# pagmerek/frave

Measured on AMD Instinct MI355X. Metric: Mpixels/s encode (transform+quant) at 4096x4096, higher is better.
Workload: dtype u8->i32

## Files before the change

### frave_amd/csrc/k4_fit.hip

```cpp
#include "gather_common.hpp"
#include "solve6.hpp"

namespace fri {
namespace {

__device__ __forceinline__ uint32_t f32_to_u32_sat(float x) {
    uint32_t r;
    asm("v_cvt_u32_f32 %0, %1" : "=v"(r) : "v"(x));
    return r;
}

struct FitArgs {
    const int32_t *coefs;
    const int32_t *pred_slots;
    const uint16_t *nbr_table;
    const uint8_t *interior;
    const uint32_t *valid_mask;
    uint32_t n_tiles;
    PredictParams pp;
    const uint32_t *pred_off;
    const uint16_t *pair_pos;
    const uint32_t *halo_list;
    unsigned long long *gram;
    unsigned long long *wtw;
    double *wtr;
    unsigned long long *out_range;
    unsigned long long *acc;
    size_t coef_stride;
    const PredictParams *params;
    PredictParams pp3[3];
    int32_t ablate;
    unsigned long long *trace;
    int32_t older_eighths;
    float *solve_params;
    float *host_params;
    unsigned long long *host_range;
    unsigned long long rows[3];
};
constexpr int kFitAccInt = 3 * 28, kFitAccDbl = kFitAccInt, kFitAccTicket = kFitAccInt + 18, kFitAccRange = kFitAccTicket + 1;
static_assert(kFitAccRange + 1 == (int)kFitAccWords, "fit accumulator layout");

template <int OFFSET>
__device__ __forceinline__ void fit2_gather(uint32_t (&g)[6], const uint32_t (&a)[6], const uint32_t (&b)[6]) {
    uint32_t lo[6], hi[6];
    asm volatile("ds_read_u16 %0, %12 offset:%24\n\t"
                 "ds_read_u16 %1, %13 offset:%24\n\t"
                 "ds_read_u16 %2, %14 offset:%24\n\t"
                 "ds_read_u16 %3, %15 offset:%24\n\t"
                 "ds_read_u16 %4, %16 offset:%24\n\t"
                 "ds_read_u16 %5, %17 offset:%24\n\t"
                 "ds_read_u16_d16_hi %6, %18 offset:%24\n\t"
                 "ds_read_u16_d16_hi %7, %19 offset:%24\n\t"
                 "ds_read_u16_d16_hi %8, %20 offset:%24\n\t"
                 "ds_read_u16_d16_hi %9, %21 offset:%24\n\t"
                 "ds_read_u16_d16_hi %10, %22 offset:%24\n\t"
                 "ds_read_u16_d16_hi %11, %23 offset:%24\n\t"
                 "s_waitcnt lgkmcnt(0)"
                 : "=&v"(lo[0]), "=&v"(lo[1]), "=&v"(lo[2]), "=&v"(lo[3]), "=&v"(lo[4]), "=&v"(lo[5]), "=&v"(hi[0]), "=&v"(hi[1]), "=&v"(hi[2]), "=&v"(hi[3]), "=&v"(hi[4]),
                   "=&v"(hi[5])
                 : "v"(a[0]), "v"(a[1]), "v"(a[2]), "v"(a[3]), "v"(a[4]), "v"(a[5]), "v"(b[0]), "v"(b[1]), "v"(b[2]), "v"(b[3]), "v"(b[4]), "v"(b[5]), "n"(OFFSET)
                 : "memory");
#pragma unroll
    for (int k = 0; k < 6; k++) g[k] = lo[k] | hi[k];
}

template <int OFFSET>
__device__ __forceinline__ void fit2_gather_floats(uint32_t (&lo)[6], uint32_t (&hi)[6], const uint32_t (&a)[6], const uint32_t (&b)[6]) {
    asm volatile("ds_read_u16_d16_hi %0, %12 offset:%24\n\t"
                 "ds_read_u16_d16_hi %1, %13 offset:%24\n\t"
                 "ds_read_u16_d16_hi %2, %14 offset:%24\n\t"
                 "ds_read_u16_d16_hi %3, %15 offset:%24\n\t"
                 "ds_read_u16_d16_hi %4, %16 offset:%24\n\t"
                 "ds_read_u16_d16_hi %5, %17 offset:%24\n\t"
                 "ds_read_u16_d16_hi %6, %18 offset:%24\n\t"
                 "ds_read_u16_d16_hi %7, %19 offset:%24\n\t"
                 "ds_read_u16_d16_hi %8, %20 offset:%24\n\t"
                 "ds_read_u16_d16_hi %9, %21 offset:%24\n\t"
                 "ds_read_u16_d16_hi %10, %22 offset:%24\n\t"
                 "ds_read_u16_d16_hi %11, %23 offset:%24\n\t"
                 "s_waitcnt lgkmcnt(0)"
                 : "=&v"(lo[0]), "=&v"(lo[1]), "=&v"(lo[2]), "=&v"(lo[3]), "=&v"(lo[4]), "=&v"(lo[5]), "=&v"(hi[0]), "=&v"(hi[1]), "=&v"(hi[2]), "=&v"(hi[3]), "=&v"(hi[4]),
                   "=&v"(hi[5])
                 : "v"(a[0]), "v"(a[1]), "v"(a[2]), "v"(a[3]), "v"(a[4]), "v"(a[5]), "v"(b[0]), "v"(b[1]), "v"(b[2]), "v"(b[3]), "v"(b[4]), "v"(b[5]), "n"(OFFSET)
                 : "memory");
}

__device__ __forceinline__ void fit2_pair_value(const uint32_t (&g)[6], uint32_t own, int (&acc)[28]) {
    s16x2 u[7];
#pragma unroll
    for (int k = 0; k < 6; k++) u[k] = __builtin_bit_cast(s16x2, g[k]);
    u[6] = __builtin_bit_cast(s16x2, own);
    int n = 0;
#pragma unroll
    for (int r0 = 0; r0 < 7; r0++)
#pragma unroll
        for (int c0 = r0; c0 < 7; c0++, n++) acc[n] = __builtin_amdgcn_sdot2(u[r0], u[c0], acc[n], false);
}

__device__ __forceinline__ void fit2_pair_width(const uint32_t (&lo)[6], const uint32_t (&hi)[6], uint32_t own, uint32_t one_bits, const float (&vp)[6], int (&acc)[28],
                                                float (&facc)[6]) {
    float fa[7], fb[7];
#pragma unroll
    for (int k = 0; k < 6; k++) fa[k] = __builtin_bit_cast(float, lo[k]), fb[k] = __builtin_bit_cast(float, hi[k]);
    fa[6] = __builtin_bit_cast(float, own << 16), fb[6] = __builtin_bit_cast(float, own & 0xFFFF0000u);
    float pa = __fmul_rn(fa[0], vp[0]), pb = __fmul_rn(fb[0], vp[0]);
#pragma unroll
    for (int k = 1; k < 6; k++) pa = __fadd_rn(pa, __fmul_rn(fa[k], vp[k])), pb = __fadd_rn(pb, __fmul_rn(fb[k], vp[k]));
    const float ra = fabsf(__fsub_rn(fa[6], pa)), rb = fabsf(__fsub_rn(fb[6], pb));
    constexpr int kD0[5] = {0, 1, 4, 1, 2}, kD1[5] = {3, 2, 5, 5, 4};
    float da[5], db[5];
#pragma unroll
    for (int j = 0; j < 5; j++) da[j] = fabsf(__fsub_rn(fa[kD0[j]], fa[kD1[j]])), db[j] = fabsf(__fsub_rn(fb[kD0[j]], fb[kD1[j]]));
    s16x2 w[6];
    w[0] = __builtin_bit_cast(s16x2, one_bits);
#pragma unroll
    for (int j = 0; j < 5; j++) {
        const uint32_t ia = __builtin_bit_cast(uint32_t, __fadd_rn(da[j], 8388608.0f)), ib = __builtin_bit_cast(uint32_t, __fadd_rn(db[j], 8388608.0f));
        w[1 + j] = __builtin_bit_cast(s16x2, __builtin_amdgcn_perm(ib, ia, 0x05040100u));
    }
    int n = 0;
#pragma unroll
    for (int r0 = 0; r0 < 6; r0++)
#pragma unroll
        for (int c0 = r0; c0 < 6; c0++, n++) acc[n] = __builtin_amdgcn_sdot2(w[r0], w[c0], acc[n], false);
    facc[0] = __fadd_rn(__fadd_rn(facc[0], ra), rb);
#pragma unroll
    for (int j = 0; j < 5; j++) {
        facc[1 + j] = __builtin_fmaf(da[j], ra, facc[1 + j]);
        facc[1 + j] = __builtin_fmaf(db[j], rb, facc[1 + j]);
    }
}

constexpr int kFit2Slot = 1024;
constexpr int kFit2Image = kPredSlots * kFit2Slot;
static_assert(kFit2Image + (kPredSide + kPredBlock) * kFit2Slot < 65536, "image + cell offset must fit a DS instruction's offset field");
struct Fit2Block {
    int4 lo, hi;
};
__device__ __forceinline__ int fit2_block_slot(int wave, int i) {
    const int c = 2 * wave + i;
    return (1 + c / kPredBlock) * kPredSide + 1 + (c % kPredBlock);
}
template <bool C16 = false>
__device__ __forceinline__ void fit2_block_load(Fit2Block &r, const int32_t *__restrict__ coefs, const int32_t *s_slot_cell, int slot, int lane, bool skip) {
    r.lo = make_int4(0, 0, 0, 0), r.hi = r.lo;
    const int cell = skip ? -1 : s_slot_cell[slot];
    if (cell >= 0) {
        if (C16) {
            r.lo = *reinterpret_cast<const int4 *>(reinterpret_cast<const int16_t *>(coefs) + (size_t)cell * kCell + 8 * lane);
        } else {
            const int4 *src = reinterpret_cast<const int4 *>(coefs + (size_t)cell * kCell + 8 * lane);
            r.lo = src[0];
            r.hi = src[1];
        }
    }
}
template <bool FLOATS>
__device__ __forceinline__ uint32_t fit2_pack(int first, int second) {
    if (!FLOATS) return __builtin_amdgcn_perm((uint32_t)second, (uint32_t)first, 0x05040100u);
    return __builtin_amdgcn_perm(__builtin_bit_cast(uint32_t, (float)(short)second), __builtin_bit_cast(uint32_t, (float)(short)first), 0x07060302u);
}
template <bool CHECK, bool FLOATS, bool C16 = false>
__device__ __forceinline__ void fit2_block_commit(const Fit2Block &r, const int32_t *s_slot_cell, uint8_t *image, int slot, int lane, uint32_t stage_pos, uint32_t *range_counter) {
    auto pk = [](int lo16, int hi16) -> uint32_t { return fit2_pack<FLOATS>(lo16, hi16); };
    if (C16) {
        static_assert(!(C16 && CHECK), "compact planes come from this library's forward kernel: nothing to check");
        auto pair = [&](int d) -> uint32_t { return FLOATS ? fit2_pack<true>(d, d >> 16) : (uint32_t)d; };
        uint8_t *dst = image + slot * kFit2Slot;
        *reinterpret_cast<uint32_t *>(dst + 4u * (stage_pos & 255u)) = pair(r.lo.x) & (lane == 0 ? 0xFFFF0000u : 0xFFFFFFFFu);
        *reinterpret_cast<uint32_t *>(dst + 4u * ((stage_pos >> 8) & 255u)) = pair(r.lo.y);
        *reinterpret_cast<uint32_t *>(dst + 4u * ((stage_pos >> 16) & 255u)) = pair(r.lo.z);
        *reinterpret_cast<uint32_t *>(dst + 4u * (stage_pos >> 24)) = pair(r.lo.w);
        return;
    }
    const int4 lo = r.lo, hi = r.hi;
    if (CHECK && s_slot_cell[slot] >= 0) {
        const int v[8] = {lo.x, lo.y, lo.z, lo.w, hi.x, hi.y, hi.z, hi.w};
        uint32_t m = 0;
#pragma unroll
        for (int j = 0; j < 8; j++) m |= v[j] == kNone ? 0u : ((uint32_t)v[j] + 256u) & 0xFFFFFE00u;
        if (__any(m != 0) && lane == 0) atomicAdd(range_counter, 1u);
    }
    uint8_t *dst = image + slot * kFit2Slot;
    *reinterpret_cast<uint32_t *>(dst + 4u * (stage_pos & 255u)) = pk(lo.x, lo.y) & (lane == 0 ? 0xFFFF0000u : 0xFFFFFFFFu);
    *reinterpret_cast<uint32_t *>(dst + 4u * ((stage_pos >> 8) & 255u)) = pk(lo.z, lo.w);
    *reinterpret_cast<uint32_t *>(dst + 4u * ((stage_pos >> 16) & 255u)) = pk(hi.x, hi.y);
    *reinterpret_cast<uint32_t *>(dst + 4u * (stage_pos >> 24)) = pk(hi.z, hi.w);
}
template <bool C16 = false>
__device__ __forceinline__ int fit2_halo_load(const int32_t *__restrict__ coefs, const int32_t *s_slot_cell, uint32_t entry, bool skip) {
    const int cell = skip ? -1 : s_slot_cell[entry & 63u];
    if (C16) return cell >= 0 ? (int)reinterpret_cast<const int16_t *>(coefs)[(size_t)cell * kCell + ((entry >> 8) & 511u)] : 0;
    return cell >= 0 ? coefs[(size_t)cell * kCell + ((entry >> 8) & 511u)] : 0;
}
template <bool FLOATS>
__device__ __forceinline__ void fit2_halo_commit(int v, uint8_t *image, uint32_t entry) {
    const uint16_t h = FLOATS ? (uint16_t)(__builtin_bit_cast(uint32_t, (float)(short)v) >> 16) : (uint16_t)v;
    *reinterpret_cast<uint16_t *>(image + (entry & 63u) * kFit2Slot + (entry >> 20)) = h;
}

template <int MODE, int IMG, int C>
__device__ __forceinline__ void fit2_cell(const int32_t *s_slot_cell, uint32_t has_bits, uint32_t interior_bits, const uint32_t *mask_word, uint32_t mask_shift, uint32_t keep, int slot0,
                                          const uint32_t (&addr)[2][6], uint32_t own_addr, const float (&vp)[6], int (&acc)[28], float (&facc)[6]) {
    constexpr int kBit = (C >> 2) * kPredSide + (C & 3);
    constexpr int kOff = IMG * kFit2Image + kBit * kFit2Slot;
    if (!((has_bits >> kBit) & 1u)) return;
    uint32_t own = *(__attribute__((address_space(3))) const uint32_t *)(uintptr_t)(own_addr + kOff) & keep;
    uint32_t one = keep & 0x00010001u;
    const bool boundary = !((interior_bits >> kBit) & 1u);
    if (MODE == 0) {
        uint32_t g[6];
        fit2_gather<kOff>(g, addr[0], addr[1]);
        if (boundary) {
            const int cell = __builtin_amdgcn_readfirstlane(s_slot_cell[slot0 + kBit]);
            const uint32_t bits = mask_word[(size_t)cell * 16] >> mask_shift;
            const uint32_t mask = ((bits & 1u) ? 0x0000FFFFu : 0u) | ((bits & 2u) ? 0xFFFF0000u : 0u);
#pragma unroll
            for (int k = 0; k < 6; k++) g[k] &= mask;
            own &= mask;
        }
        fit2_pair_value(g, own, acc);
    } else {
        uint32_t lo[6], hi[6];
        fit2_gather_floats<kOff>(lo, hi, addr[0], addr[1]);
        if (boundary) {
            const int cell = __builtin_amdgcn_readfirstlane(s_slot_cell[slot0 + kBit]);
            const uint32_t bits = mask_word[(size_t)cell * 16] >> mask_shift;
            const uint32_t first = (bits & 1u) ? 0xFFFFFFFFu : 0u, second = (bits & 2u) ? 0xFFFFFFFFu : 0u;
#pragma unroll
            for (int k = 0; k < 6; k++) lo[k] &= first, hi[k] &= second;
            own &= (first & 0xFFFFu) | (second << 16), one &= (first & 0xFFFFu) | (second << 16);
        }
        fit2_pair_width(lo, hi, own, one, vp, acc, facc);
    }
    asm volatile("" ::: "memory");
}
template <int MODE, int IMG, int C0>
__device__ __forceinline__ void fit2_cells(const int32_t *s_slot_cell, uint32_t has_bits, uint32_t interior_bits, const uint32_t *mask_word, uint32_t mask_shift, uint32_t keep, int slot0,
                                           const uint32_t (&addr)[2][6], uint32_t own_addr, const float (&vp)[6], int (&acc)[28], float (&facc)[6]) {
    fit2_cell<MODE, IMG, C0 + 0>(s_slot_cell, has_bits, interior_bits, mask_word, mask_shift, keep, slot0, addr, own_addr, vp, acc, facc);
    fit2_cell<MODE, IMG, C0 + 1>(s_slot_cell, has_bits, interior_bits, mask_word, mask_shift, keep, slot0, addr, own_addr, vp, acc, facc);
    fit2_cell<MODE, IMG, C0 + 2>(s_slot_cell, has_bits, interior_bits, mask_word, mask_shift, keep, slot0, addr, own_addr, vp, acc, facc);
    fit2_cell<MODE, IMG, C0 + 3>(s_slot_cell, has_bits, interior_bits, mask_word, mask_shift, keep, slot0, addr, own_addr, vp, acc, facc);
}

template <int NI>
__device__ __forceinline__ void fit2_wave_sums(int (&acc)[28], int group, int lane, unsigned long long (*s_int)[28]) {
    int r[NI];
#pragma unroll
    for (int k = 0; k < NI; k++) r[k] = acc[k], acc[k] = 0;
#pragma unroll
    for (int k = 0; k < NI; k++) r[k] += __builtin_amdgcn_update_dpp(0, r[k], 0xB1, 0xF, 0xF, true);
#pragma unroll
    for (int k = 0; k < NI; k++) r[k] += __builtin_amdgcn_update_dpp(0, r[k], 0x4E, 0xF, 0xF, true);
#pragma unroll
    for (int k = 0; k < NI; k++) r[k] += __builtin_amdgcn_update_dpp(0, r[k], 0x141, 0xF, 0xF, true);
#pragma unroll
    for (int k = 0; k < NI; k++) r[k] += __builtin_amdgcn_update_dpp(0, r[k], 0x140, 0xF, 0xF, true);
    if ((lane & 15) == 0) {
        unsigned long long *const mine = &s_int[(lane >> 4) * 3 + group][0];
#pragma unroll
        for (int k = 0; k < NI; k++) atomicAdd(mine + k, (unsigned long long)(long long)r[k]);
    }
}

constexpr int kFitFixBits = 20;
__device__ __forceinline__ unsigned long long fit_f32_to_fixed(float v0, bool &saturated) {
    saturated = saturated || !(v0 < 16777216.0f);
    const float v = fminf(v0, 16777216.0f);
    const float t = __builtin_truncf(v);
    const uint32_t hi = f32_to_u32_sat(t);
    const uint32_t lo = f32_to_u32_sat((v - t) * (float)(1u << kFitFixBits));
    return ((unsigned long long)hi << kFitFixBits) + lo;
}

template <int MODE>
__device__ __attribute__((noinline)) void fit2_tail_solve(const long long *sums_int, const double *sums_dbl, unsigned long long rows, Solve6Work *w, float *params,
                                                          float *host_params) {
    float out[6];
    if (MODE == 0)
        fit_value_group(sums_int, out, *w);
    else
        fit_width_group(sums_int, sums_dbl, rows, out, *w);
#pragma unroll
    for (int k = 0; k < 6; k++) params[k] = out[k];
    if (host_params) {
#pragma unroll
        for (int k = 0; k < 6; k++) host_params[k] = out[k];
    }
}

template <int MODE, bool CHECK, bool C16 = false>
__global__ void __launch_bounds__(kPredThreads, 4) fit_accumulate_kernel2(const FitArgs a0) {
    constexpr int NI = MODE == 0 ? 28 : 21;
    const uint32_t plane = blockIdx.y;
    const int32_t *const coefs = C16 ? reinterpret_cast<const int32_t *>(reinterpret_cast<const int16_t *>(a0.coefs) + plane * a0.coef_stride) : a0.coefs + plane * a0.coef_stride;
    unsigned long long *const accp = a0.acc + (size_t)plane * kFitShards * kFitAccWords;
    unsigned long long *const accs = accp + (size_t)(blockIdx.x % kFitShards) * kFitAccWords;
    PredictParams pp;
    if (a0.params)
        pp = a0.params[plane];
    else if (plane == 0)
        pp = a0.pp3[0];
    else if (plane == 1)
        pp = a0.pp3[1];
    else
        pp = a0.pp3[2];
    __shared__ __attribute__((aligned(16))) uint8_t s_cells[2 * kFit2Image];
    __shared__ int32_t s_slot_cell[2][kPredSlots];
    __shared__ uint32_t s_slot_bits[2][2];
    __shared__ uint32_t s_flag, s_range;
    __shared__ unsigned long long s_int[4 * 3][28];
    __shared__ unsigned long long s_fix[16 * 3][6];
    __shared__ double s_dbl[3][6];
    const int tid = threadIdx.x, lane = tid & 63;
    const int wave = __builtin_amdgcn_readfirstlane(tid >> 6);
    const int pg = wave & 3, half = wave >> 2;
    const int n0 = pg == 0 ? 128 + 2 * lane : pg == 1 ? 2 * lane : 256 + 4 * lane + 2 * (pg & 1);
    const int ablate = ablate_flags(a0.ablate);
    PredTileWalk walk(a0.n_tiles);
    if (a0.older_eighths > 0 && gridDim.x >= 16u && gridDim.x % 16u == 0u) {
        const uint32_t per_xcd = gridDim.x / 8u, pairs = per_xcd / 2u;
        const uint32_t xcd = blockIdx.x % 8u, in_xcd = blockIdx.x / 8u, pair = in_xcd % pairs, younger = in_xcd / pairs;
        const uint32_t lo = (uint32_t)((uint64_t)a0.n_tiles * xcd / 8u), hi = (uint32_t)((uint64_t)a0.n_tiles * (xcd + 1u) / 8u);
        const uint32_t n_pair = lo + pair < hi ? (hi - lo - pair + pairs - 1u) / pairs : 0u;
        const uint32_t n_older = min(n_pair, (n_pair * (uint32_t)a0.older_eighths + 3u) / 8u);
        walk.step = pairs;
        walk.first = lo + pair + (younger ? n_older * pairs : 0u);
        walk.end = younger ? hi : min(hi, lo + pair + n_older * pairs);
        if (walk.first > walk.end) walk.first = walk.end;
    }
    auto slot_entry = [&](uint32_t t) {
        uint32_t off = (uint32_t)tid * 4u;
        asm volatile("" : "+v"(off));
        return *reinterpret_cast<const int32_t *>(reinterpret_cast<const uint8_t *>(a0.pred_slots + (size_t)t * kPredSlots) + off);
    };
    const u32x4 off_a = reinterpret_cast<const u32x4 *>(a0.pred_off)[n0], off_b = reinterpret_cast<const u32x4 *>(a0.pred_off)[n0 + 1];
    const uint32_t own_pos = a0.pair_pos[n0 >> 1];
    const uint32_t halo_e0 = a0.halo_list[tid], halo_e1 = a0.halo_list[tid + kPredThreads];
    const uint32_t stage_pos = (uint32_t)a0.pair_pos[4 * lane] | (uint32_t)a0.pair_pos[4 * lane + 1] << 8 | (uint32_t)a0.pair_pos[4 * lane + 2] << 16 | (uint32_t)a0.pair_pos[4 * lane + 3] << 24;
    int first_raw = -1, next_raw = -1;
    if (tid < kPredSlots && walk.first < walk.end) first_raw = slot_entry(walk.first);
    if (tid < kPredSlots && walk.first + walk.step < walk.end) next_raw = slot_entry(walk.first + walk.step);
    __builtin_amdgcn_sched_barrier(0);
    if (tid < 4 * 3 * 28) (&s_int[0][0])[tid] = 0;
    if (tid < 16 * 18) (&s_fix[0][0])[tid] = 0ull;
    if (tid == 0) s_range = 0;
    trace_stamp(a0.trace, blockIdx.x, 0, tid);

    const int group = pg == 0 ? 1 : pg == 1 ? 2 : 0;
    const int slot0 = (1 + 2 * half) * kPredSide + 1;
    const uint32_t cells_lds = (uint32_t)(uintptr_t)(__attribute__((address_space(3))) uint8_t *)s_cells;
    uint32_t addr[2][6];
#pragma unroll
    for (int j = 0; j < 2; j++) {
        const u32x4 o = j == 0 ? off_a : off_b;
        const uint32_t rel[3] = {o.x, o.y, o.z};
#pragma unroll
        for (int k = 0; k < 6; k++) {
            const int r = (int)(short)((rel[k >> 1] >> (16 * (k & 1))) & 0xFFFFu);
            addr[j][k] = cells_lds + (uint32_t)(slot0 * kFit2Slot + (r == 0x7FFF ? 0 : r));
        }
    }
    uint32_t own_addr = cells_lds + (uint32_t)(slot0 * kFit2Slot) + 4u * own_pos;
    if (n0 == 0) {
#pragma unroll
        for (int j = 0; j < 2; j++)
#pragma unroll
            for (int k = 0; k < 6; k++) addr[j][k] = cells_lds + (uint32_t)(slot0 * kFit2Slot);
    }
    const uint32_t *const mask_word = a0.valid_mask + (n0 >> 5);
    const uint32_t mask_shift = n0 & 31;
    const uint32_t keep = n0 == 0 ? 0u : 0xFFFFFFFFu;
    float vp[6];
#pragma unroll
    for (int k = 0; k < 6; k++) vp[k] = group == 0 ? pp.value[0][k] : group == 1 ? pp.value[1][k] : pp.value[2][k];
    int acc[28];
    unsigned long long fx[6];
#pragma unroll
    for (int k = 0; k < 28; k++) acc[k] = 0;
#pragma unroll
    for (int k = 0; k < 6; k++) fx[k] = 0ull;
    bool fx_saturated = false;
    int tiles_since_flush = 0, trace_it = 0;
    const int block_a = fit2_block_slot(wave, 0), block_b = fit2_block_slot(wave, 1);

    uint32_t tile = walk.first;
    static_assert((kPredBlock * kPredSide + kPredBlock) < 32 && kPredSlots <= 64, "the block slots' bits fit one word; the slot table is written by one wave");
    auto slot_table = [&](int img, int raw) {
        s_slot_cell[img][tid] = pred_slot_cell(raw);
        const unsigned long long has = __ballot(pred_slot_cell(raw) >= 0), interior = __ballot(pred_slot_interior(raw));
        if (tid == 0) s_slot_bits[img][0] = (uint32_t)has, s_slot_bits[img][1] = (uint32_t)interior;
    };
#define FRI_FIT2_PHASE(IMG)                                                                                                                       \
    {                                                                                                                                            \
               \
                                                          \
        if (tid < kPredSlots) slot_table(IMG ^ 1, tile + walk.step < walk.end ? next_raw : -1);                                                  \
        __syncthreads();                                                                                                                         \
        float facc[6] = {0.f, 0.f, 0.f, 0.f, 0.f, 0.f};                                                                                          \
        const uint32_t has_bits = (uint32_t)__builtin_amdgcn_readfirstlane((int)s_slot_bits[IMG][0]) >> slot0;                                   \
        const uint32_t interior_bits = (uint32_t)__builtin_amdgcn_readfirstlane((int)s_slot_bits[IMG][1]) >> slot0;                              \
        {                                                                                                                                        \
            Fit2Block st;                                                                                                                        \
            fit2_block_load<C16>(st, coefs, s_slot_cell[IMG ^ 1], block_a, lane, ablate & 2);                                                         \
            const int hv = fit2_halo_load<C16>(coefs, s_slot_cell[IMG ^ 1], halo_e0, ablate & 2);                                                     \
            if (tid < kPredSlots && tile + 2 * walk.step < walk.end) next_raw = slot_entry(tile + 2 * walk.step);                                 \
            if (!(ablate & 1)) fit2_cells<MODE, IMG, 0>(s_slot_cell[IMG], has_bits, interior_bits, mask_word, mask_shift, keep, slot0, addr, own_addr, vp, acc, facc); \
            fit2_block_commit<CHECK, MODE == 1, C16>(st, s_slot_cell[IMG ^ 1], s_cells + (IMG ^ 1) * kFit2Image, block_a, lane, stage_pos, &s_range);                              \
            fit2_halo_commit<MODE == 1>(hv, s_cells + (IMG ^ 1) * kFit2Image, halo_e0);                                                                     \
        }                                                                                                                                        \
        {                                                                                                                                        \
            Fit2Block st;                                                                                                                        \
            fit2_block_load<C16>(st, coefs, s_slot_cell[IMG ^ 1], block_b, lane, ablate & 2);                                                         \
            const int hv = fit2_halo_load<C16>(coefs, s_slot_cell[IMG ^ 1], halo_e1, ablate & 2);                                                     \
            if (!(ablate & 1)) fit2_cells<MODE, IMG, 4>(s_slot_cell[IMG], has_bits, interior_bits, mask_word, mask_shift, keep, slot0, addr, own_addr, vp, acc, facc); \
            fit2_block_commit<CHECK, MODE == 1, C16>(st, s_slot_cell[IMG ^ 1], s_cells + (IMG ^ 1) * kFit2Image, block_b, lane, stage_pos, &s_range);                              \
            fit2_halo_commit<MODE == 1>(hv, s_cells + (IMG ^ 1) * kFit2Image, halo_e1);                                                                     \
        }                                                                                                                                        \
        if (MODE == 1) {                                                                                                                         \
            _Pragma("unroll") for (int k = 0; k < 6; k++) fx[k] += fit_f32_to_fixed(facc[k], fx_saturated);                                     \
        }                                                                                                                                        \
        if (++tiles_since_flush >= 16) {             \
            fit2_wave_sums<NI>(acc, group, lane, s_int);                                                                                         \
            tiles_since_flush = 0;                                                                                                               \
        }                                                                                                                                        \
        __syncthreads();                                                                                                                         \
        trace_stamp(a0.trace, blockIdx.x, 2 + trace_it++, tid);                                                                                  \
        tile += walk.step;                                                                                                                       \
    }
    if (tile < walk.end) {
        if (tid < kPredSlots) slot_table(0, first_raw);
        __syncthreads();
        {
            Fit2Block sa, sb;
            fit2_block_load<C16>(sa, coefs, s_slot_cell[0], block_a, lane, false);
            fit2_block_load<C16>(sb, coefs, s_slot_cell[0], block_b, lane, false);
            const int h0 = fit2_halo_load<C16>(coefs, s_slot_cell[0], halo_e0, false), h1 = fit2_halo_load<C16>(coefs, s_slot_cell[0], halo_e1, false);
            fit2_block_commit<CHECK, MODE == 1, C16>(sa, s_slot_cell[0], s_cells, block_a, lane, stage_pos, &s_range);
            fit2_block_commit<CHECK, MODE == 1, C16>(sb, s_slot_cell[0], s_cells, block_b, lane, stage_pos, &s_range);
            fit2_halo_commit<MODE == 1>(h0, s_cells, halo_e0);
            fit2_halo_commit<MODE == 1>(h1, s_cells, halo_e1);
        }
        __syncthreads();
        trace_stamp(a0.trace, blockIdx.x, 1, tid);
        while (true) {
            FRI_FIT2_PHASE(0)
            if (tile >= walk.end) break;
            FRI_FIT2_PHASE(1)
            if (tile >= walk.end) break;
        }
    }
#undef FRI_FIT2_PHASE
    trace_stamp(a0.trace, blockIdx.x, 13, tid);
    fit2_wave_sums<NI>(acc, group, lane, s_int);
    if (MODE == 1) {
        unsigned long long *const mine = &s_fix[(lane & 15) * 3 + group][0];
#pragma unroll
        for (int k = 0; k < 6; k++) atomicAdd(mine + k, fx[k]);
        if (__any(fx_saturated) && lane == 0) atomicAdd(&s_range, 1u);
    }
    __syncthreads();
    if (tid < 3 * NI) {
        const int gg = tid / NI, k = tid % NI;
        __hip_atomic_fetch_add(accs + tid, (s_int[gg][k] + s_int[3 + gg][k]) + (s_int[6 + gg][k] + s_int[9 + gg][k]), __ATOMIC_RELAXED, __HIP_MEMORY_SCOPE_AGENT);
    }
    if (MODE == 1 && tid < 18) {
        unsigned long long v = 0;
#pragma unroll
        for (int c = 0; c < 16; c++) v += (&s_fix[0][0])[c * 18 + tid];
        __hip_atomic_fetch_add(accs + kFitAccDbl + tid, v, __ATOMIC_RELAXED, __HIP_MEMORY_SCOPE_AGENT);
    }
    if (tid == 0 && s_range) __hip_atomic_fetch_add(accp + kFitAccRange, (unsigned long long)s_range, __ATOMIC_RELAXED, __HIP_MEMORY_SCOPE_AGENT);
    wait_for_own_memory_ops_then_barrier();
    if (tid == 0) s_flag = __hip_atomic_fetch_add(accp + kFitAccTicket, 1ull, __ATOMIC_RELAXED, __HIP_MEMORY_SCOPE_AGENT) == gridDim.x - 1 ? 1u : 0u;
    __syncthreads();
    trace_exit(a0.trace, blockIdx.x, tid);
    if (s_flag == 0) return;
    if (tid >= 64) return;
    unsigned long long *const out_int = (MODE == 0 ? a0.gram : a0.wtw) + (size_t)plane * 3 * NI;
    for (int i = tid; i < 3 * NI; i += 64) {
        unsigned long long part[kFitShards], sum = 0;
#pragma unroll
        for (uint32_t sh = 0; sh < kFitShards; sh++) part[sh] = __hip_atomic_load(accp + sh * kFitAccWords + i, __ATOMIC_RELAXED, __HIP_MEMORY_SCOPE_AGENT);
#pragma unroll
        for (uint32_t sh = 0; sh < kFitShards; sh++) {
            sum += part[sh];
            __hip_atomic_store(accp + sh * kFitAccWords + i, 0ull, __ATOMIC_RELAXED, __HIP_MEMORY_SCOPE_AGENT);
        }
        out_int[i] = sum;
        s_int[i / NI][i % NI] = sum;
    }
    if (MODE == 1 && tid < 18) {
        unsigned long long part[kFitShards], total = 0;
#pragma unroll
        for (uint32_t sh = 0; sh < kFitShards; sh++) part[sh] = __hip_atomic_load(accp + sh * kFitAccWords + kFitAccDbl + tid, __ATOMIC_RELAXED, __HIP_MEMORY_SCOPE_AGENT);
#pragma unroll
        for (uint32_t sh = 0; sh < kFitShards; sh++) {
            total += part[sh];
            __hip_atomic_store(accp + sh * kFitAccWords + kFitAccDbl + tid, 0ull, __ATOMIC_RELAXED, __HIP_MEMORY_SCOPE_AGENT);
        }
        const double sum = (double)total * (1.0 / (double)(1ull << kFitFixBits));
        a0.wtr[(size_t)plane * 18 + tid] = sum;
        (&s_dbl[0][0])[tid] = sum;
    }
    if (tid == 0) {
        const unsigned long long r = __hip_atomic_exchange(accp + kFitAccRange, 0ull, __ATOMIC_RELAXED, __HIP_MEMORY_SCOPE_AGENT);
        if (a0.out_range) a0.out_range[plane] = r;
        if (a0.host_range) a0.host_range[plane] = r;
        __hip_atomic_store(accp + kFitAccTicket, 0ull, __ATOMIC_RELAXED, __HIP_MEMORY_SCOPE_AGENT);
    }
    if (!a0.solve_params) return;
    __builtin_amdgcn_fence(__ATOMIC_RELEASE, "wavefront");
    __builtin_amdgcn_wave_barrier();
    __builtin_amdgcn_fence(__ATOMIC_ACQUIRE, "wavefront");
    if (tid < 3) {
        static_assert(3 * sizeof(Solve6Work) <= 2 * kFit2Image, "the solve's workspace lives in the cell images");
        const unsigned long long rows = tid == 0 ? a0.rows[0] : tid == 1 ? a0.rows[1] : a0.rows[2];
        const size_t at = (size_t)plane * (sizeof(PredictParams) / sizeof(float)) + (MODE ? 18 : 0) + tid * 6;
        fit2_tail_solve<MODE>(reinterpret_cast<const long long *>(s_int[tid]), s_dbl[tid], rows, reinterpret_cast<Solve6Work *>(s_cells) + tid, a0.solve_params + at,
                              a0.host_params ? a0.host_params + at : nullptr);
    }
}

struct SolveArgs {
    const unsigned long long *sums_int;
    const double *sums_dbl;
    float *params;
    uint32_t n_planes;
    unsigned long long rows[3];
    float *host_params;
    const unsigned long long *range;
    unsigned long long *host_range;
};
constexpr uint32_t kSolveThreads = 32;
template <int MODE>
__global__ void __launch_bounds__(kSolveThreads) fit_solve_kernel(const SolveArgs a) {
    __shared__ Solve6Work s_work[kSolveThreads];
    Solve6Work &w = s_work[threadIdx.x];
    const uint32_t t = blockIdx.x * kSolveThreads + threadIdx.x;
    if (t >= a.n_planes * 3u) return;
    const uint32_t plane = t / 3u, g = t % 3u;
    float *out = a.params + (size_t)plane * (sizeof(PredictParams) / sizeof(float)) + (MODE ? 18 : 0) + g * 6;
    if (MODE == 0) {
        fit_value_group(reinterpret_cast<const long long *>(a.sums_int) + ((size_t)plane * 3 + g) * 28, out, w);
    } else {
        const unsigned long long rows = g == 0 ? a.rows[0] : g == 1 ? a.rows[1] : a.rows[2];
        fit_width_group(reinterpret_cast<const long long *>(a.sums_int) + ((size_t)plane * 3 + g) * 21, a.sums_dbl + ((size_t)plane * 3 + g) * 6, rows, out, w);
    }
    if (a.host_params) {
        float *h = a.host_params + (out - a.params);
#pragma unroll
        for (int k = 0; k < 6; k++) h[k] = out[k];
        if (g == 0 && a.range && a.host_range) a.host_range[plane] = a.range[plane];
    }
}

}

hipError_t launch_fit_solve(int mode, uint32_t n_planes, const unsigned long long *sums_int, const double *sums_dbl, const unsigned long long rows[3], float *params,
                            hipStream_t stream, float *host_params, const unsigned long long *range, unsigned long long *host_range) {
    if (!n_planes || !sums_int || !params || (mode == 1 && !sums_dbl)) return hipErrorInvalidValue;
    SolveArgs a{};
    a.sums_int = sums_int;
    a.sums_dbl = sums_dbl;
    a.params = params;
    a.n_planes = n_planes;
    a.host_params = host_params, a.range = range, a.host_range = host_range;
    for (int g = 0; g < 3; g++) a.rows[g] = rows ? rows[g] : 0;
    const uint32_t blocks = (n_planes * 3u + kSolveThreads - 1u) / kSolveThreads;
    (void)hipGetLastError();
    if (mode == 0)
        hipLaunchKernelGGL(fit_solve_kernel<0>, dim3(blocks), dim3(kSolveThreads), 0, stream, a);
    else
        hipLaunchKernelGGL(fit_solve_kernel<1>, dim3(blocks), dim3(kSolveThreads), 0, stream, a);
    return hipGetLastError();
}

hipError_t launch_fit_accumulate(const DevicePlan &p, unsigned long long *acc, int mode, const PredBatch &b, unsigned long long *sums_int, double *sums_dbl,
                                 unsigned long long *out_of_range, hipStream_t stream, const FitSolve *solve, int trust) {
    if (!acc || !b.n_planes || b.n_planes > 65535u) return hipErrorInvalidValue;
    FitArgs a{};
    if (b.coefs16 && trust != kPredForwardOutput) return hipErrorInvalidValue;
    a.coefs = b.coefs16 ? reinterpret_cast<const int32_t *>(b.coefs16) : b.coefs;
    a.coef_stride = b.coef_stride;
    a.params = b.params;
    for (int k = 0; k < 3; k++) a.pp3[k] = b.pp[k];
    a.pred_slots = p.pred_slots;
    a.nbr_table = p.nbr_table;
    a.pred_off = p.gather_off;
    a.pair_pos = p.pair_pos;
    a.halo_list = p.halo_list;
    a.interior = p.interior;
    a.valid_mask = p.valid_mask;
    a.n_tiles = p.n_pred_tiles;
    a.acc = acc;
    a.gram = sums_int;
    a.wtw = sums_int;
    a.wtr = sums_dbl;
    a.out_range = out_of_range;
    if (solve) {
        if (!solve->params) return hipErrorInvalidValue;
        a.solve_params = solve->params, a.host_params = solve->host_params, a.host_range = solve->host_range;
        for (int g = 0; g < 3; g++) a.rows[g] = solve->rows[g];
    }
    a.ablate = p.k4_ablate;
    a.trace = p.trace;
    a.older_eighths = b.n_planes == 1 && p.hist_blocks <= p.n_pred_tiles ? p.k4_older_eighths : 0;
    uint32_t blocks = p.n_pred_tiles < p.hist_blocks ? p.n_pred_tiles : p.hist_blocks;
    if (b.n_planes > 1) {
        const uint32_t share = (p.n_pred_tiles + 7) / 8, eighth = p.hist_blocks / 8 ? p.hist_blocks / 8 : 1;
        blocks = share < eighth ? eighth : share;
        if (blocks > p.hist_blocks) blocks = p.hist_blocks;
        if (blocks > p.n_pred_tiles) blocks = p.n_pred_tiles;
    }
    if (!blocks) blocks = 1;
    (void)hipGetLastError();
    const bool check = trust != kPredForwardOutput;
    void (*kern)(const FitArgs) = mode == 0 ? (check ? fit_accumulate_kernel2<0, true> : fit_accumulate_kernel2<0, false>) : (check ? fit_accumulate_kernel2<1, true> : fit_accumulate_kernel2<1, false>);
    if (b.coefs16) kern = mode == 0 ? fit_accumulate_kernel2<0, false, true> : fit_accumulate_kernel2<1, false, true>;
    hipLaunchKernelGGL(kern, dim3(blocks, b.n_planes), dim3(kPredThreads), 0, stream, a);
    return hipGetLastError();
}

}
```

### frave_amd/csrc/solve6.hpp

```cpp
#pragma once
#include <cmath>

#if defined(__HIPCC__)
#define FRI_HD __host__ __device__
#else
#define FRI_HD
#endif

namespace fri {

struct Solve6Work {
    double m[6][6], y[6], x[6];
    double l[6][6], d[6], inv[6], z[6];
    double a[6][6], v[6][6];
};

#if defined(__HIP_DEVICE_COMPILE__)
#define FRI_SOLVE_STAGE() asm volatile("" ::: "memory")
#else
#define FRI_SOLVE_STAGE() ((void)0)
#endif

FRI_HD inline void solve6(Solve6Work &w) {
    {
        double dmax = 0.0;
#pragma unroll
        for (int i = 0; i < 6; i++) dmax = w.m[i][i] > dmax ? w.m[i][i] : dmax;
        bool ok = dmax > 0.0 && dmax < 1.0e300;
        FRI_SOLVE_STAGE();
#pragma unroll
        for (int j = 0; j < 6; j++) {
            double dj = w.m[j][j];
#pragma unroll
            for (int k = 0; k < j; k++) dj -= w.l[j][k] * w.l[j][k] * w.d[k];
            ok = ok && dj > 1e-8 * dmax;
            w.d[j] = dj;
            w.inv[j] = 1.0 / dj;
#pragma unroll
            for (int i = j + 1; i < 6; i++) {
                double t = w.m[i][j];
#pragma unroll
                for (int k = 0; k < j; k++) t -= w.l[i][k] * w.l[j][k] * w.d[k];
                w.l[i][j] = t * w.inv[j];
            }
            FRI_SOLVE_STAGE();
        }
        if (ok) {
#pragma unroll
            for (int i = 0; i < 6; i++) {
                double t = w.y[i];
#pragma unroll
                for (int k = 0; k < i; k++) t -= w.l[i][k] * w.z[k];
                w.z[i] = t;
            }
            FRI_SOLVE_STAGE();
#pragma unroll
            for (int i = 5; i >= 0; i--) {
                double t = w.z[i] * w.inv[i];
#pragma unroll
                for (int k = i + 1; k < 6; k++) t -= w.l[k][i] * w.x[k];
                w.x[i] = t;
            }
            return;
        }
    }
#pragma unroll 1
    for (int i = 0; i < 6; i++)
#pragma unroll 1
        for (int j = 0; j < 6; j++) {
            w.a[i][j] = w.m[i][j];
            w.v[i][j] = i == j ? 1.0 : 0.0;
        }
#pragma unroll 1
    for (int sweep = 0; sweep < 60; sweep++) {
        double off = 0.0;
#pragma unroll 1
        for (int i = 0; i < 6; i++)
#pragma unroll 1
            for (int j = i + 1; j < 6; j++) off += w.a[i][j] * w.a[i][j];
        if (!(off >= 1e-300)) break;
#pragma unroll 1
        for (int pp = 0; pp < 6; pp++)
#pragma unroll 1
            for (int q = pp + 1; q < 6; q++) {
                const double apq = w.a[pp][q];
                if ((apq < 0 ? -apq : apq) < 1e-300) continue;
                const double theta = (w.a[q][q] - w.a[pp][pp]) / (2.0 * apq);
                const double t = (theta >= 0 ? 1.0 : -1.0) / ((theta < 0 ? -theta : theta) + sqrt(theta * theta + 1.0));
                const double c = 1.0 / sqrt(t * t + 1.0), sn = t * c;
#pragma unroll 1
                for (int k = 0; k < 6; k++) {
                    const double akp = w.a[k][pp], akq = w.a[k][q];
                    w.a[k][pp] = c * akp - sn * akq;
                    w.a[k][q] = sn * akp + c * akq;
                }
#pragma unroll 1
                for (int k = 0; k < 6; k++) {
                    const double apk = w.a[pp][k], aqk = w.a[q][k];
                    w.a[pp][k] = c * apk - sn * aqk;
                    w.a[q][k] = sn * apk + c * aqk;
                }
#pragma unroll 1
                for (int k = 0; k < 6; k++) {
                    const double vkp = w.v[k][pp], vkq = w.v[k][q];
                    w.v[k][pp] = c * vkp - sn * vkq;
                    w.v[k][q] = sn * vkp + c * vkq;
                }
            }
    }
    double lmax = 0.0;
#pragma unroll 1
    for (int i = 0; i < 6; i++) lmax = w.a[i][i] > lmax ? w.a[i][i] : lmax;
#pragma unroll 1
    for (int k = 0; k < 6; k++) w.x[k] = 0.0;
#pragma unroll 1
    for (int i = 0; i < 6; i++) {
        if (!(w.a[i][i] > 1e-12 * lmax)) continue;
        double proj = 0.0;
#pragma unroll 1
        for (int k = 0; k < 6; k++) proj += w.v[k][i] * w.y[k];
#pragma unroll 1
        for (int k = 0; k < 6; k++) w.x[k] += w.v[k][i] * proj / w.a[i][i];
    }
}

FRI_HD inline int tri_index(int i, int j, int n) {
    if (i > j) {
        const int t = i;
        i = j;
        j = t;
    }
    return i * n - i * (i - 1) / 2 + (j - i);
}

FRI_HD inline void fit_value_group(const long long *gram, float *out , Solve6Work &w) {
    for (int i = 0; i < 6; i++) {
        w.y[i] = (double)gram[tri_index(i, 6, 7)];
        for (int j = 0; j < 6; j++) w.m[i][j] = (double)gram[tri_index(i, j, 7)];
    }
    solve6(w);
    for (int k = 0; k < 6; k++) out[k] = (float)w.x[k];
}

FRI_HD inline void fit_width_group(const long long *wtw, const double *wtr, unsigned long long rows, float *out , Solve6Work &w) {
    for (int i = 0; i < 6; i++) {
        w.y[i] = wtr[i];
        for (int j = 0; j < 6; j++) w.m[i][j] = (double)wtw[tri_index(i, j, 6)];
    }
    w.m[0][0] += (double)rows - (double)wtw[0];
    solve6(w);
    for (int k = 0; k < 6; k++) out[k] = (float)w.x[k];
}

}
```

Before: 915,100.

## Parallelize fit tail reduction per wave and solve 6x6 LDLT across lanes

The last-block tail of the fit accumulator is restructured. Each of three waves now reduces its own group's shard sums, and a fourth wave handles the range and ticket reset. The 6x6 normal-equation LDLT solve is spread across six lanes using readlane broadcasts, with the serial min-norm Jacobi fallback kept for ill-conditioned systems. The goal is to shorten the serial single-thread tail that runs after the grid-wide ticket. In exchange the code is more complex, per-wave pointer setup is hoisted before the barrier, and trace-tail hooks are added.

```diff
diff --git a/frave_amd/csrc/k4_fit.hip b/frave_amd/csrc/k4_fit.hip
--- a/frave_amd/csrc/k4_fit.hip
+++ b/frave_amd/csrc/k4_fit.hip
@@ -31,6 +31,7 @@
     PredictParams pp3[3];
     int32_t ablate;
     unsigned long long *trace;
+    unsigned long long *trace_tail;
     int32_t older_eighths;
     float *solve_params;
     float *host_params;
@@ -274,20 +275,49 @@
     return ((unsigned long long)hi << kFitFixBits) + lo;
 }
 
+struct Ldl6Wave {
+    Ldl6Lane s;
+    int i;
+    template <class F>
+    __device__ __forceinline__ void each(F f) { f(s, i); }
+    static __device__ __forceinline__ double from_lane(double v, int src) {
+        const int lo = __builtin_amdgcn_readlane(__double2loint(v), src), hi = __builtin_amdgcn_readlane(__double2hiint(v), src);
+        return __hiloint2double(hi, lo);
+    }
+    __device__ __forceinline__ double diag(int j) const { return from_lane(s.t[j], j); }
+    __device__ __forceinline__ double lower(int src, int j) const { return from_lane(s.l[j], src); }
+    __device__ __forceinline__ double rhs(int src) const { return from_lane(s.y, src); }
+};
+
 template <int MODE>
-__device__ __attribute__((noinline)) void fit2_tail_solve(const long long *sums_int, const double *sums_dbl, unsigned long long rows, Solve6Work *w, float *params,
-                                                          float *host_params) {
-    float out[6];
+__device__ __attribute__((noinline)) void fit2_tail_min_norm(const long long *sums_int, const double *sums_dbl, unsigned long long rows, Solve6Work *w, float *params,
+                                                             float *host_params) {
     if (MODE == 0)
-        fit_value_group(sums_int, out, *w);
+        fit_value_system(sums_int, *w);
     else
-        fit_width_group(sums_int, sums_dbl, rows, out, *w);
-#pragma unroll
-    for (int k = 0; k < 6; k++) params[k] = out[k];
-    if (host_params) {
-#pragma unroll
-        for (int k = 0; k < 6; k++) host_params[k] = out[k];
-    }
+        fit_width_system(sums_int, sums_dbl, rows, *w);
+    solve6_min_norm(*w);
+#pragma unroll 1
+    for (int k = 0; k < 6; k++) {
+        const float out = (float)w->x[k];
+        params[k] = out;
+        if (host_params) host_params[k] = out;
+    }
+}
+
+template <int MODE>
+__device__ __attribute__((noinline)) bool fit2_tail_solve(const long long *sums_int, const double *sums_dbl, unsigned long long rows, float *params, float *host_params, int lane) {
+    Ldl6Wave g;
+    g.i = lane;
+    if (MODE == 0)
+        ldl6_load_value(g.s, lane, sums_int);
+    else
+        ldl6_load_width(g.s, lane, sums_int, sums_dbl, rows);
+    if (!ldl6_lane_schedule(g)) return false;
+    const float out = (float)g.s.y;
+    params[lane] = out;
+    if (host_params) host_params[lane] = out;
+    return true;
 }
 
 template <int MODE, bool CHECK, bool C16 = false>
@@ -472,55 +502,63 @@
         __hip_atomic_fetch_add(accs + kFitAccDbl + tid, v, __ATOMIC_RELAXED, __HIP_MEMORY_SCOPE_AGENT);
     }
     if (tid == 0 && s_range) __hip_atomic_fetch_add(accp + kFitAccRange, (unsigned long long)s_range, __ATOMIC_RELAXED, __HIP_MEMORY_SCOPE_AGENT);
+    const int grp = wave < 3 ? wave : 0;
+    unsigned long long *out_int = (MODE == 0 ? a0.gram : a0.wtw) + (size_t)plane * 3 * NI + grp * NI;
+    double *out_dbl = MODE == 1 ? a0.wtr + (size_t)plane * 18 + grp * 6 : nullptr;
+    const size_t solve_at = (size_t)plane * (sizeof(PredictParams) / sizeof(float)) + (MODE ? 18 : 0) + grp * 6;
+    float *solve_dst = a0.solve_params ? a0.solve_params + solve_at : nullptr, *solve_host = a0.host_params ? a0.host_params + solve_at : nullptr;
+    unsigned long long solve_rows = grp == 0 ? a0.rows[0] : grp == 1 ? a0.rows[1] : a0.rows[2];
+    asm volatile("" : "+s"(out_int), "+s"(out_dbl), "+s"(solve_dst), "+s"(solve_host), "+s"(solve_rows));
     wait_for_own_memory_ops_then_barrier();
     if (tid == 0) s_flag = __hip_atomic_fetch_add(accp + kFitAccTicket, 1ull, __ATOMIC_RELAXED, __HIP_MEMORY_SCOPE_AGENT) == gridDim.x - 1 ? 1u : 0u;
     __syncthreads();
     trace_exit(a0.trace, blockIdx.x, tid);
     if (s_flag == 0) return;
-    if (tid >= 64) return;
-    unsigned long long *const out_int = (MODE == 0 ? a0.gram : a0.wtw) + (size_t)plane * 3 * NI;
-    for (int i = tid; i < 3 * NI; i += 64) {
+    if (wave > 3) return;
+    if (wave == 3) {
+        if (lane == 0) {
+            const unsigned long long r = __hip_atomic_exchange(accp + kFitAccRange, 0ull, __ATOMIC_RELAXED, __HIP_MEMORY_SCOPE_AGENT);
+            if (a0.out_range) a0.out_range[plane] = r;
+            if (a0.host_range) a0.host_range[plane] = r;
+            __hip_atomic_store(accp + kFitAccTicket, 0ull, __ATOMIC_RELAXED, __HIP_MEMORY_SCOPE_AGENT);
+        }
+        return;
+    }
+    unsigned long long *const tail = kTraceBuild && a0.trace && a0.trace_tail && plane == 0 ? a0.trace_tail + MODE * kTraceSlots : nullptr;
+    trace_stamp(tail, 0, 1, tid);
+    if (lane < NI + (MODE == 1 ? 6 : 0)) {
+        const bool fixed = MODE == 1 && lane >= NI;
+        unsigned long long *const src = accp + (fixed ? kFitAccDbl + wave * 6 + (lane - NI) : wave * NI + lane);
         unsigned long long part[kFitShards], sum = 0;
 #pragma unroll
-        for (uint32_t sh = 0; sh < kFitShards; sh++) part[sh] = __hip_atomic_load(accp + sh * kFitAccWords + i, __ATOMIC_RELAXED, __HIP_MEMORY_SCOPE_AGENT);
+        for (uint32_t sh = 0; sh < kFitShards; sh++) part[sh] = __hip_atomic_load(src + sh * kFitAccWords, __ATOMIC_RELAXED, __HIP_MEMORY_SCOPE_AGENT);
 #pragma unroll
         for (uint32_t sh = 0; sh < kFitShards; sh++) {
             sum += part[sh];
-            __hip_atomic_store(accp + sh * kFitAccWords + i, 0ull, __ATOMIC_RELAXED, __HIP_MEMORY_SCOPE_AGENT);
-        }
-        out_int[i] = sum;
-        s_int[i / NI][i % NI] = sum;
-    }
-    if (MODE == 1 && tid < 18) {
-        unsigned long long part[kFitShards], total = 0;
-#pragma unroll
-        for (uint32_t sh = 0; sh < kFitShards; sh++) part[sh] = __hip_atomic_load(accp + sh * kFitAccWords + kFitAccDbl + tid, __ATOMIC_RELAXED, __HIP_MEMORY_SCOPE_AGENT);
-#pragma unroll
-        for (uint32_t sh = 0; sh < kFitShards; sh++) {
-            total += part[sh];
-            __hip_atomic_store(accp + sh * kFitAccWords + kFitAccDbl + tid, 0ull, __ATOMIC_RELAXED, __HIP_MEMORY_SCOPE_AGENT);
-        }
-        const double sum = (double)total * (1.0 / (double)(1ull << kFitFixBits));
-        a0.wtr[(size_t)plane * 18 + tid] = sum;
-        (&s_dbl[0][0])[tid] = sum;
-    }
-    if (tid == 0) {
-        const unsigned long long r = __hip_atomic_exchange(accp + kFitAccRange, 0ull, __ATOMIC_RELAXED, __HIP_MEMORY_SCOPE_AGENT);
-        if (a0.out_range) a0.out_range[plane] = r;
-        if (a0.host_range) a0.host_range[plane] = r;
-        __hip_atomic_store(accp + kFitAccTicket, 0ull, __ATOMIC_RELAXED, __HIP_MEMORY_SCOPE_AGENT);
-    }
-    if (!a0.solve_params) return;
+            __hip_atomic_store(src + sh * kFitAccWords, 0ull, __ATOMIC_RELAXED, __HIP_MEMORY_SCOPE_AGENT);
+        }
+        if (!fixed) {
+            out_int[lane] = sum;
+            s_int[wave][lane] = sum;
+        } else {
+            const double total = (double)sum * (1.0 / (double)(1ull << kFitFixBits));
+            out_dbl[lane - NI] = total;
+            s_dbl[wave][lane - NI] = total;
+        }
+    }
+    trace_stamp(tail, 0, 2, tid);
+    if (!solve_dst) return;
     __builtin_amdgcn_fence(__ATOMIC_RELEASE, "wavefront");
     __builtin_amdgcn_wave_barrier();
     __builtin_amdgcn_fence(__ATOMIC_ACQUIRE, "wavefront");
-    if (tid < 3) {
-        static_assert(3 * sizeof(Solve6Work) <= 2 * kFit2Image, "the solve's workspace lives in the cell images");
-        const unsigned long long rows = tid == 0 ? a0.rows[0] : tid == 1 ? a0.rows[1] : a0.rows[2];
-        const size_t at = (size_t)plane * (sizeof(PredictParams) / sizeof(float)) + (MODE ? 18 : 0) + tid * 6;
-        fit2_tail_solve<MODE>(reinterpret_cast<const long long *>(s_int[tid]), s_dbl[tid], rows, reinterpret_cast<Solve6Work *>(s_cells) + tid, a0.solve_params + at,
-                              a0.host_params ? a0.host_params + at : nullptr);
-    }
+    if (lane < 6) {
+        static_assert(3 * sizeof(Solve6Work) <= 2 * kFit2Image, "the fallback's workspace lives in the (now idle) cell images");
+        const long long *const sums = reinterpret_cast<const long long *>(s_int[wave]);
+        if (!fit2_tail_solve<MODE>(sums, s_dbl[wave], solve_rows, solve_dst, solve_host, lane) && lane == 0)
+            fit2_tail_min_norm<MODE>(sums, s_dbl[wave], solve_rows, reinterpret_cast<Solve6Work *>(s_cells) + wave, solve_dst, solve_host);
+    }
+    trace_stamp(tail, 0, 3, tid);
+    if (tail && tid == 0) tail[0] = blockIdx.x, tail[4] = a0.trace[(size_t)blockIdx.x * kTraceSlots + 13], tail[5] = a0.trace[(size_t)blockIdx.x * kTraceSlots + 15];
 }
 
 struct SolveArgs {
@@ -606,6 +644,7 @@
     }
     a.ablate = p.k4_ablate;
     a.trace = p.trace;
+    a.trace_tail = nullptr;
     a.older_eighths = b.n_planes == 1 && p.hist_blocks <= p.n_pred_tiles ? p.k4_older_eighths : 0;
     uint32_t blocks = p.n_pred_tiles < p.hist_blocks ? p.n_pred_tiles : p.hist_blocks;
     if (b.n_planes > 1) {
@@ -615,6 +654,7 @@
         if (blocks > p.n_pred_tiles) blocks = p.n_pred_tiles;
     }
     if (!blocks) blocks = 1;
+    if (p.trace && (size_t)blocks + 2 <= p.n_wg) a.trace_tail = p.trace + (size_t)blocks * kTraceSlots;
     (void)hipGetLastError();
     const bool check = trust != kPredForwardOutput;
     void (*kern)(const FitArgs) = mode == 0 ? (check ? fit_accumulate_kernel2<0, true> : fit_accumulate_kernel2<0, false>) : (check ? fit_accumulate_kernel2<1, true> : fit_accumulate_kernel2<1, false>);
diff --git a/frave_amd/csrc/solve6.hpp b/frave_amd/csrc/solve6.hpp
--- a/frave_amd/csrc/solve6.hpp
+++ b/frave_amd/csrc/solve6.hpp
@@ -21,7 +21,7 @@
 #define FRI_SOLVE_STAGE() ((void)0)
 #endif
 
-FRI_HD inline void solve6(Solve6Work &w) {
+FRI_HD inline bool solve6_ldlt(Solve6Work &w) {
     {
         double dmax = 0.0;
 #pragma unroll
@@ -61,9 +61,13 @@
                 for (int k = i + 1; k < 6; k++) t -= w.l[k][i] * w.x[k];
                 w.x[i] = t;
             }
-            return;
-        }
-    }
+            return true;
+        }
+    }
+    return false;
+}
+
+FRI_HD inline void solve6_min_norm(Solve6Work &w) {
 #pragma unroll 1
     for (int i = 0; i < 6; i++)
 #pragma unroll 1
@@ -124,6 +128,10 @@
     }
 }
 
+FRI_HD inline void solve6(Solve6Work &w) {
+    if (!solve6_ldlt(w)) solve6_min_norm(w);
+}
+
 FRI_HD inline int tri_index(int i, int j, int n) {
     if (i > j) {
         const int t = i;
@@ -133,23 +141,158 @@
     return i * n - i * (i - 1) / 2 + (j - i);
 }
 
+#define FRI_ROLLED _Pragma("unroll 1")
+FRI_HD inline void fit_value_system(const long long *gram, Solve6Work &w) {
+    FRI_ROLLED
+    for (int i = 0; i < 6; i++) {
+        w.y[i] = (double)gram[tri_index(i, 6, 7)];
+        FRI_ROLLED
+        for (int j = 0; j < 6; j++) w.m[i][j] = (double)gram[tri_index(i, j, 7)];
+    }
+}
+FRI_HD inline void fit_width_system(const long long *wtw, const double *wtr, unsigned long long rows, Solve6Work &w) {
+    FRI_ROLLED
+    for (int i = 0; i < 6; i++) {
+        w.y[i] = wtr[i];
+        FRI_ROLLED
+        for (int j = 0; j < 6; j++) w.m[i][j] = (double)wtw[tri_index(i, j, 6)];
+    }
+    w.m[0][0] += (double)rows - (double)wtw[0];
+}
+
+#undef FRI_ROLLED
+
 FRI_HD inline void fit_value_group(const long long *gram, float *out , Solve6Work &w) {
-    for (int i = 0; i < 6; i++) {
-        w.y[i] = (double)gram[tri_index(i, 6, 7)];
-        for (int j = 0; j < 6; j++) w.m[i][j] = (double)gram[tri_index(i, j, 7)];
-    }
+    fit_value_system(gram, w);
     solve6(w);
     for (int k = 0; k < 6; k++) out[k] = (float)w.x[k];
 }
 
 FRI_HD inline void fit_width_group(const long long *wtw, const double *wtr, unsigned long long rows, float *out , Solve6Work &w) {
-    for (int i = 0; i < 6; i++) {
-        w.y[i] = wtr[i];
-        for (int j = 0; j < 6; j++) w.m[i][j] = (double)wtw[tri_index(i, j, 6)];
-    }
-    w.m[0][0] += (double)rows - (double)wtw[0];
+    fit_width_system(wtw, wtr, rows, w);
     solve6(w);
     for (int k = 0; k < 6; k++) out[k] = (float)w.x[k];
 }
 
-}
+struct Ldl6Lane {
+    double t[6];
+    double l[6];
+    double y;
+    double inv;
+};
+
+FRI_HD inline void ldl6_load(Ldl6Lane &s, int i, const Solve6Work &w) {
+#pragma unroll
+    for (int j = 0; j < 6; j++) s.t[j] = w.m[i][j];
+    s.y = w.y[i];
+}
+FRI_HD inline void ldl6_load_value(Ldl6Lane &s, int i, const long long *gram) {
+#pragma unroll
+    for (int j = 0; j < 6; j++) s.t[j] = (double)gram[tri_index(i, j, 7)];
+    s.y = (double)gram[tri_index(i, 6, 7)];
+}
+FRI_HD inline void ldl6_load_width(Ldl6Lane &s, int i, const long long *wtw, const double *wtr, unsigned long long rows) {
+#pragma unroll
+    for (int j = 0; j < 6; j++) s.t[j] = (double)wtw[tri_index(i, j, 6)];
+    if (i == 0) s.t[0] += (double)rows - (double)wtw[0];
+    s.y = wtr[i];
+}
+
+template <class G>
+FRI_HD inline bool ldl6_lane_schedule(G &g) {
+    double dmax = 0.0;
+#pragma unroll
+    for (int i = 0; i < 6; i++) {
+        const double mii = g.diag(i);
+        dmax = mii > dmax ? mii : dmax;
+    }
+    bool ok = dmax > 0.0 && dmax < 1.0e300;
+#pragma unroll
+    for (int j = 0; j < 6; j++) {
+        const double dj = g.diag(j);
+        ok = ok && dj > 1e-8 * dmax;
+        const double inv = 1.0 / dj;
+        g.each([&](Ldl6Lane &s, int i) {
+            s.l[j] = s.t[j] * inv;
+            if (i == j) s.inv = inv;
+        });
+#pragma unroll
+        for (int c = j + 1; c < 6; c++) {
+            const double lcj = g.lower(c, j);
+            g.each([&](Ldl6Lane &s, int i) {
+                s.t[c] -= s.l[j] * lcj * dj;
+            });
+        }
+    }
+    if (!ok) return false;
+#pragma unroll
+    for (int k = 0; k < 6; k++) {
+        const double zk = g.rhs(k);
+        g.each([&](Ldl6Lane &s, int i) {
+            if (i > k) s.y -= s.l[k] * zk;
+        });
+    }
+    g.each([&](Ldl6Lane &s, int) { s.y = s.y * s.inv; });
+    double x[6];
+#pragma unroll
+    for (int r = 5; r >= 0; r--) {
+        double t = g.rhs(r);
+#pragma unroll
+        for (int k = r + 1; k < 6; k++) t -= g.lower(k, r) * x[k];
+        x[r] = t;
+        g.each([&](Ldl6Lane &s, int i) {
+            if (i == r) s.y = t;
+        });
+    }
+    return true;
+}
+
+struct Ldl6Emulation {
+    Ldl6Lane s[6];
+    template <class F>
+    FRI_HD void each(F f) {
+        for (int i = 0; i < 6; i++) f(s[i], i);
+    }
+    FRI_HD double diag(int j) const { return s[j].t[j]; }
+    FRI_HD double lower(int src, int j) const { return s[src].l[j]; }
+    FRI_HD double rhs(int src) const { return s[src].y; }
+};
+
+inline bool solve6_lanes(Solve6Work &w) {
+    Ldl6Emulation g{};
+    for (int i = 0; i < 6; i++) ldl6_load(g.s[i], i, w);
+    if (ldl6_lane_schedule(g)) {
+        for (int i = 0; i < 6; i++) w.x[i] = g.s[i].y;
+        return true;
+    }
+    solve6_min_norm(w);
+    return false;
+}
+inline bool fit_value_group_lanes(const long long *gram, float *out , Solve6Work &w) {
+    Ldl6Emulation g{};
+    for (int i = 0; i < 6; i++) ldl6_load_value(g.s[i], i, gram);
+    const bool ldlt = ldl6_lane_schedule(g);
+    if (ldlt) {
+        for (int i = 0; i < 6; i++) w.x[i] = g.s[i].y;
+    } else {
+        fit_value_system(gram, w);
+        solve6_min_norm(w);
+    }
+    for (int k = 0; k < 6; k++) out[k] = (float)w.x[k];
+    return ldlt;
+}
+inline bool fit_width_group_lanes(const long long *wtw, const double *wtr, unsigned long long rows, float *out , Solve6Work &w) {
+    Ldl6Emulation g{};
+    for (int i = 0; i < 6; i++) ldl6_load_width(g.s[i], i, wtw, wtr, rows);
+    const bool ldlt = ldl6_lane_schedule(g);
+    if (ldlt) {
+        for (int i = 0; i < 6; i++) w.x[i] = g.s[i].y;
+    } else {
+        fit_width_system(wtw, wtr, rows, w);
+        solve6_min_norm(w);
+    }
+    for (int k = 0; k < 6; k++) out[k] = (float)w.x[k];
+    return ldlt;
+}
+
+}
```

Result: no change. 908,800 (-0.7%).
